# FifthEpoch/longcat-video-tta

Hardware: AMD Instinct MI355X
Metric: denoised latent frames/sec (49x720p, 50-step CFG denoise) (higher is better)
Workload: dtype bf16; 1 GPU; K3: 49x720p (13 latent frames, 46 800 tokens); DiT 48 blocks x 4096 hidden, CFG 4.0, 50-step flow-match Euler, no conditioning frames; depth=48, parallelism=dp1

## Files before the change

longcat-video-tta_amd/csrc/attn_fwd_w64.hip:

```cpp
#include "attn_common.h"
#include <type_traits>

struct AttnFwdW64Params : AttnFwdLead {
  float scale;
  int gx, xcd_remap;
};

template <int I, int N, class F>
__device__ __forceinline__ void w64_static_for(F&& f) {
  if constexpr (I < N) { f(std::integral_constant<int, I>{}); w64_static_for<I + 1, N>(f); }
}
enum : unsigned char { W64_NONE, W64_EXP, W64_ADD, W64_PACK, W64_LRUN, W64_VOFF, W64_MAX, W64_HMAX, W64_BALLOT, W64_M0, W64_DMA };
struct W64Op { unsigned char kind, b, e; };
constexpr int W64_SLOTS = 6;
constexpr W64Op W64_P1[32][W64_SLOTS] = {
  {{W64_EXP, 0, 0}, {W64_EXP, 1, 0}},
  {{W64_EXP, 0, 1}},
  {{W64_PACK, 0, 0}, {W64_ADD, 0, 1}, {W64_EXP, 1, 1}, {W64_EXP, 0, 2}},
  {{W64_ADD, 0, 2}, {W64_PACK, 1, 0}, {W64_ADD, 1, 1}, {W64_EXP, 1, 2}},
  {{W64_ADD, 1, 2}, {W64_EXP, 0, 3}, {W64_EXP, 1, 3}},
  {{W64_PACK, 0, 1}, {W64_ADD, 0, 3}, {W64_PACK, 1, 1}, {W64_ADD, 1, 3}, {W64_EXP, 0, 4}},
  {{W64_ADD, 0, 4}, {W64_EXP, 1, 4}, {W64_EXP, 0, 5}},
  {{W64_PACK, 0, 2}, {W64_ADD, 0, 5}, {W64_ADD, 1, 4}, {W64_EXP, 1, 5}},
  {{W64_PACK, 1, 2}, {W64_ADD, 1, 5}, {W64_EXP, 0, 6}, {W64_EXP, 1, 6}},
  {{W64_ADD, 0, 6}, {W64_ADD, 1, 6}, {W64_EXP, 0, 7}},
  {{W64_VOFF, 0, 0}, {W64_PACK, 0, 3}, {W64_ADD, 0, 7}, {W64_EXP, 1, 7}, {W64_EXP, 0, 8}},
  {{W64_VOFF, 1, 0}, {W64_ADD, 0, 8}, {W64_PACK, 1, 3}, {W64_ADD, 1, 7}, {W64_EXP, 1, 8}},
  {{W64_VOFF, 2, 0}, {W64_ADD, 1, 8}, {W64_EXP, 0, 9}, {W64_EXP, 1, 9}},
  {{W64_VOFF, 3, 0}, {W64_PACK, 0, 4}, {W64_ADD, 0, 9}, {W64_PACK, 1, 4}, {W64_ADD, 1, 9}, {W64_EXP, 0, 10}},
  {{W64_VOFF, 4, 0}, {W64_ADD, 0, 10}, {W64_EXP, 1, 10}, {W64_EXP, 0, 11}},
  {{W64_VOFF, 5, 0}, {W64_PACK, 0, 5}, {W64_ADD, 0, 11}, {W64_ADD, 1, 10}, {W64_EXP, 1, 11}},
  {{W64_VOFF, 6, 0}, {W64_PACK, 1, 5}, {W64_ADD, 1, 11}, {W64_EXP, 0, 12}, {W64_EXP, 1, 12}},
  {{W64_VOFF, 7, 0}, {W64_ADD, 0, 12}, {W64_ADD, 1, 12}, {W64_EXP, 0, 13}},
  {{W64_PACK, 0, 6}, {W64_ADD, 0, 13}, {W64_EXP, 1, 13}, {W64_EXP, 0, 14}},
  {{W64_ADD, 0, 14}, {W64_PACK, 1, 6}, {W64_ADD, 1, 13}, {W64_EXP, 1, 14}},
  {{W64_ADD, 1, 14}, {W64_EXP, 0, 15}, {W64_EXP, 1, 15}},
  {{W64_PACK, 0, 7}, {W64_ADD, 0, 15}, {W64_PACK, 1, 7}, {W64_ADD, 1, 15}, {W64_EXP, 0, 16}},
  {{W64_ADD, 0, 16}, {W64_EXP, 1, 16}, {W64_EXP, 0, 17}},
  {{W64_PACK, 0, 8}, {W64_ADD, 0, 17}, {W64_ADD, 1, 16}, {W64_EXP, 1, 17}},
  {{W64_PACK, 1, 8}, {W64_ADD, 1, 17}, {W64_EXP, 0, 18}, {W64_EXP, 1, 18}},
  {{W64_ADD, 0, 18}, {W64_ADD, 1, 18}, {W64_EXP, 0, 19}},
  {{W64_PACK, 0, 9}, {W64_ADD, 0, 19}, {W64_EXP, 1, 19}, {W64_EXP, 0, 20}},
  {{W64_ADD, 0, 20}, {W64_PACK, 1, 9}, {W64_ADD, 1, 19}, {W64_EXP, 1, 20}},
  {{W64_ADD, 1, 20}, {W64_EXP, 0, 21}, {W64_EXP, 1, 21}},
  {{W64_PACK, 0, 10}, {W64_ADD, 0, 21}, {W64_PACK, 1, 10}, {W64_ADD, 1, 21}, {W64_EXP, 0, 22}},
  {{W64_ADD, 0, 22}, {W64_EXP, 1, 22}, {W64_EXP, 0, 23}},
  {{W64_PACK, 0, 11}, {W64_ADD, 0, 23}, {W64_ADD, 1, 22}, {W64_EXP, 1, 23}},
};
constexpr W64Op W64_P2[32][W64_SLOTS] = {
  {{W64_M0, 0, 0}, {W64_PACK, 1, 11}, {W64_ADD, 1, 23}, {W64_EXP, 0, 24}, {W64_DMA, 0, 0}},
  {{W64_ADD, 0, 24}, {W64_EXP, 1, 24}},
  {{W64_M0, 1, 0}, {W64_ADD, 1, 24}, {W64_EXP, 0, 25}, {W64_DMA, 1, 0}},
  {{W64_PACK, 0, 12}, {W64_ADD, 0, 25}},
  {{W64_M0, 2, 0}, {W64_EXP, 1, 25}, {W64_DMA, 2, 0}},
  {{W64_PACK, 1, 12}, {W64_ADD, 1, 25}, {W64_EXP, 0, 26}},
  {{W64_M0, 3, 0}, {W64_ADD, 0, 26}, {W64_DMA, 3, 0}},
  {{W64_EXP, 1, 26}},
  {{W64_M0, 4, 0}, {W64_ADD, 1, 26}, {W64_MAX, 0, 0}, {W64_EXP, 0, 27}, {W64_DMA, 4, 0}},
  {{W64_PACK, 0, 13}, {W64_ADD, 0, 27}, {W64_MAX, 1, 0}},
  {{W64_M0, 5, 0}, {W64_MAX, 0, 1}, {W64_EXP, 1, 27}, {W64_DMA, 5, 0}},
  {{W64_PACK, 1, 13}, {W64_ADD, 1, 27}, {W64_MAX, 1, 1}, {W64_EXP, 0, 28}},
  {{W64_M0, 6, 0}, {W64_ADD, 0, 28}, {W64_MAX, 0, 2}, {W64_EXP, 1, 28}, {W64_DMA, 6, 0}},
  {{W64_ADD, 1, 28}, {W64_MAX, 1, 2}},
  {{W64_M0, 7, 0}, {W64_MAX, 0, 3}, {W64_EXP, 0, 29}, {W64_DMA, 7, 0}},
  {{W64_PACK, 0, 14}, {W64_ADD, 0, 29}, {W64_MAX, 1, 3}, {W64_EXP, 1, 29}},
  {{W64_PACK, 1, 14}, {W64_ADD, 1, 29}, {W64_MAX, 0, 4}},
  {{W64_MAX, 1, 4}, {W64_EXP, 0, 30}},
  {{W64_ADD, 0, 30}, {W64_MAX, 0, 5}, {W64_EXP, 1, 30}},
  {{W64_ADD, 1, 30}, {W64_MAX, 1, 5}},
  {{W64_MAX, 0, 6}, {W64_EXP, 0, 31}},
  {{W64_PACK, 0, 15}, {W64_ADD, 0, 31}, {W64_MAX, 1, 6}, {W64_EXP, 1, 31}},
  {{W64_PACK, 1, 15}, {W64_ADD, 1, 31}, {W64_LRUN, 0, 0}, {W64_MAX, 0, 7}},
  {{W64_LRUN, 1, 0}, {W64_MAX, 1, 7}},
  {{W64_HMAX, 0, 0}},
  {{W64_HMAX, 1, 0}},
  {{W64_BALLOT, 0, 0}},
  {{W64_BALLOT, 1, 0}},
  {},
  {},
  {},
  {},
};
constexpr int w64_op_cost(W64Op o) {
  return o.kind == W64_EXP ? 8 : o.kind == W64_PACK ? 5 : o.kind == W64_MAX ? 8 : o.kind == W64_HMAX ? 20 :
         o.kind == W64_NONE ? 0 : 4;
}
constexpr int w64_read_cost(int phase, int i) {
  return !(i & 1) || i > 29 ? 0 : ((phase == 1 && i >= 27) || (phase == 2 && i <= 25)) ? 12 : 8;
}
constexpr bool w64_table_ok(const W64Op (&t)[32][W64_SLOTS], int phase, int max_cyc, int max_exp) {
  for (int i = 0; i < 32; ++i) {
    int c = w64_read_cost(phase, i), ex = 0;
    for (int s = 0; s < W64_SLOTS; ++s) { c += w64_op_cost(t[i][s]); ex += t[i][s].kind == W64_EXP; }
    if (c > max_cyc || ex > max_exp) return false;
  }
  return true;
}
constexpr bool w64_table_complete() {
  int exp_at[2][32] = {}, add_at[2][32] = {}, pack_at[2][16] = {}, n = 0;
  for (int b = 0; b < 2; ++b) for (int e = 0; e < 32; ++e) { exp_at[b][e] = -1; add_at[b][e] = -1; }
  for (int b = 0; b < 2; ++b) for (int m = 0; m < 16; ++m) pack_at[b][m] = -1;
  for (int g = 0; g < 64; ++g)
    for (int s = 0; s < W64_SLOTS; ++s) {
      const W64Op o = g < 32 ? W64_P1[g][s] : W64_P2[g - 32][s];
      const int at = 8 * g + s;
      if (o.kind == W64_EXP) { if (exp_at[o.b][o.e] >= 0) return false; exp_at[o.b][o.e] = at; ++n; }
      if (o.kind == W64_ADD) { if (o.e == 0 || exp_at[o.b][o.e] < 0 || (o.e > 1 && add_at[o.b][o.e - 1] < 0)) return false; add_at[o.b][o.e] = at; }
      if (o.kind == W64_PACK) { if (exp_at[o.b][2 * o.e] < 0 || exp_at[o.b][2 * o.e + 1] < 0) return false; pack_at[o.b][o.e] = at; }
      if (o.kind == W64_LRUN && add_at[o.b][31] < 0) return false;
    }
  for (int b = 0; b < 2; ++b)
    for (int m = 0; m < 16; ++m)
      if (pack_at[b][m] < 0 || pack_at[b][m] >= 8 * (32 + 8 * (m / 4) + b - 1) + W64_SLOTS) return false;
  return n == 64;
}
static_assert(w64_table_complete(), "attn_fwd_w64 gap table: an exp, add or pack is missing, doubled or out of order");
static_assert(w64_table_ok(W64_P1, 1, 38, 2) && w64_table_ok(W64_P2, 2, 37, 1), "attn_fwd_w64 gap table over its budget");

template <bool GUARD>
__device__ __forceinline__ void mfma_s(f32x16& c, const bf16x8& a, const bf16x8& b) {
  if constexpr (GUARD) asm volatile("s_nop 3\n\tv_mfma_f32_32x32x16_bf16 %0, %1, %2, %0" : "+v"(c) : "v"(a), "a"(b));
  else asm volatile("v_mfma_f32_32x32x16_bf16 %0, %1, %2, %0" : "+v"(c) : "v"(a), "a"(b));
}
template <bool GUARD>
__device__ __forceinline__ void mfma_s_first(f32x16& d, const f32x16& c, const bf16x8& a, const bf16x8& b) {
  if constexpr (GUARD) asm volatile("s_nop 3\n\tv_mfma_f32_32x32x16_bf16 %0, %2, %3, %1" : "=&v"(d) : "v"(c), "v"(a), "a"(b));
  else asm volatile("v_mfma_f32_32x32x16_bf16 %0, %2, %3, %1" : "=&v"(d) : "v"(c), "v"(a), "a"(b));
}
template <bool GUARD>
__device__ __forceinline__ void mfma_o(f32x16& c, const bf16x8& a, const bf16x8& b) {
  if constexpr (GUARD) asm volatile("s_nop 3\n\tv_mfma_f32_32x32x16_bf16 %0, %1, %2, %0" : "+a"(c) : "v"(a), "v"(b));
  else asm volatile("v_mfma_f32_32x32x16_bf16 %0, %1, %2, %0" : "+a"(c) : "v"(a), "v"(b));
}

#define SCW(S, nb, j) (S[(j) >> 4][nb][(j) & 15])

__global__ __launch_bounds__(256) void attn_fwd_w64_kernel(const AttnFwdW64Params p) {
  constexpr int TILE = 64 * 256;
  extern __shared__ __attribute__((aligned(16))) unsigned char smem[];
  lds_u8* lds = (lds_u8*)smem;
  constexpr int V_REGION = 2 * TILE;

  const int tid = threadIdx.x;
  const int lane = tid & 63;
  const int wave = __builtin_amdgcn_readfirstlane(tid >> 6);
  const int r = lane & 31, h = lane >> 5;
  int qb, head;
  int64_t b;
  ATTN_BLOCK_DECODE(p, qb, head, b);
  const int64_t q0 = (int64_t)qb * 256 + wave * 64;
  const int nt = (int)((p.d.Nk + 63) / 64);
  const bool ragged = (p.d.Nk & 63) != 0;
  const char* kbase_u = lcv_uniform_ptr(p.k + b * p.d.k_sb + (int64_t)head * p.d.k_sh);
  const char* vbase_u = lcv_uniform_ptr(p.v + b * p.d.v_sb + (int64_t)head * p.d.v_sh);

  auto dma_row_of = [&](int ln, int i) { return 16 * wave + 4 * i + (ln >> 4); };
  auto dma_colb_of = [&](int ln, int i) {
    const int row = dma_row_of(ln, i);
    return 16 * ((ln & 15) ^ attn_swz(row));
  };
  unsigned koff[4], voff[4];
#pragma unroll
  for (int i = 0; i < 4; ++i) {
    koff[i] = (unsigned)(dma_row_of(lane, i) * p.d.k_sn * 2 + dma_colb_of(lane, i));
    voff[i] = (unsigned)(dma_row_of(lane, i) * p.d.v_sn * 2 + dma_colb_of(lane, i));
  }
  auto last_off = [&](int i, int64_t sn) {
    const int ln = lane_now();
    int64_t row = (int64_t)(nt - 1) * 64 + dma_row_of(ln, i);
    if (row > p.d.Nk - 1) row = p.d.Nk - 1;
    return (unsigned)(row * sn * 2 + dma_colb_of(ln, i));
  };
  const unsigned lds_wave = (unsigned)(uintptr_t)lds + (unsigned)wave * 4096u;
  auto dma_one = [&](int which, int i, int dst_tile, int tile, bool known_full) __attribute__((always_inline)) {
    const int64_t sn = which ? p.d.v_sn : p.d.k_sn;
    const char* base = which ? vbase_u : kbase_u;
    unsigned off = which ? voff[i] : koff[i];
    if (!known_full && tile == nt - 1) off = last_off(i, sn);
    else base += (int64_t)tile * (128 * sn);
    asm volatile("s_mov_b32 m0, %2\n\ts_nop 0\n\tglobal_load_lds_dwordx4 %0, %1"
                 :: "v"(off), "s"(base), "s"(lds_wave + (unsigned)dst_tile + 1024u * i) : "memory", "m0");
  };
  auto dma_m0 = [&](int i, int dst_tile) __attribute__((always_inline)) {
    asm volatile("s_mov_b32 m0, %0" :: "s"(lds_wave + (unsigned)dst_tile + 1024u * i) : "memory", "m0");
  };
  auto dma_req = [&](int which, int i, int tile, bool known_full) __attribute__((always_inline)) {
    const int64_t sn = which ? p.d.v_sn : p.d.k_sn;
    const char* base = which ? vbase_u : kbase_u;
    unsigned off = which ? voff[i] : koff[i];
    if (!known_full && tile == nt - 1) off = last_off(i, sn);
    else base += (int64_t)tile * (128 * sn);
    asm volatile("global_load_lds_dwordx4 %0, %1" :: "v"(off), "s"(base) : "memory");
  };
  auto dma_tile = [&](int which, int dst_tile, int tile) __attribute__((always_inline)) {
#pragma unroll
    for (int i = 0; i < 4; ++i) dma_one(which, i, dst_tile, tile, false);
  };
  constexpr int KOP = 0, VOP = 1;
  auto dma_wait_and_barrier = [&]() { asm volatile("s_waitcnt vmcnt(0)\n\ts_barrier" ::: "memory"); };

  int k_off[8];
  int v_off[2][4];
  auto set_read_offsets = [&](int ln, int slot) {
    const int rr = ln & 31, hh = ln >> 5;
    const int kfz = ((rr & 3) << 2) | ((rr >> 2) & 3);
#pragma unroll
    for (int ks = 0; ks < 8; ++ks) k_off[ks] = 256 * rr + 16 * ((2 * ks + hh) ^ kfz);
    const int q4 = (ln >> 2) & 3, p4 = ln & 3, g1 = (ln >> 4) & 1;
#pragma unroll
    for (int half = 0; half < 2; ++half)
#pragma unroll
      for (int d = 0; d < 4; ++d)
        v_off[half][d] = (int)(unsigned)(uintptr_t)lds + V_REGION + slot * TILE + 256 * (4 * hh + 8 * half + q4) + 8 * (p4 & 1) + 64 * (d ^ q4) +
                         16 * ((2 * g1 + (p4 >> 1)) ^ (hh + 2 * half));
  };
  set_read_offsets(lane, 2);
  auto read_k = [&](const lds_u8* kb, int f) __attribute__((always_inline)) -> bf16x8 {
    return *reinterpret_cast<const AS3 bf16x8*>(kb + (f & 1) * 32 * 256 + k_off[f >> 1]);
  };
  auto read_v = [&](int g) __attribute__((always_inline)) -> bf16x8 {
    const s16x4 lo = __builtin_amdgcn_ds_read_tr16_b64_v4i16((AS3 s16x4*)(uintptr_t)(unsigned)(v_off[0][g & 3] + 4096 * (g >> 2)));
    const s16x4 hi = __builtin_amdgcn_ds_read_tr16_b64_v4i16((AS3 s16x4*)(uintptr_t)(unsigned)(v_off[1][g & 3] + 4096 * (g >> 2)));
    return __builtin_bit_cast(bf16x8, __builtin_shufflevector(lo, hi, 0, 1, 2, 3, 4, 5, 6, 7));
  };

  bf16x8 qf[2][8];
#pragma unroll
  for (int nb = 0; nb < 2; ++nb) {
    int64_t qrow = q0 + 32 * nb + r;
    if (qrow > p.d.Nq - 1) qrow = p.d.Nq - 1;
    const bf16_t* qp = p.q + b * p.d.q_sb + qrow * p.d.q_sn + (int64_t)head * p.d.q_sh + 8 * h;
#pragma unroll
    for (int ks = 0; ks < 8; ++ks) qf[nb][ks] = *reinterpret_cast<const bf16x8*>(qp + 16 * ks);
  }
#pragma unroll
  for (int nb = 0; nb < 2; ++nb)
#pragma unroll
    for (int ks = 0; ks < 8; ++ks) asm volatile("" : "+a"(qf[nb][ks]));

  f32x16 oacc[2][4];
#pragma unroll
  for (int nb = 0; nb < 2; ++nb)
#pragma unroll
    for (int d = 0; d < 4; ++d) {
#pragma unroll
      for (int e = 0; e < 16; ++e) oacc[nb][d][e] = 0.f;
      asm volatile("" : "+a"(oacc[nb][d]));
    }
  float m_run[2] = {0.f, 0.f}, l_run[2] = {0.f, 0.f};
  f32x16 minit[2];
#pragma unroll
  for (int nb = 0; nb < 2; ++nb)
#pragma unroll
    for (int e = 0; e < 16; ++e) minit[nb][e] = 0.f;
  f32x16 sa[2][2], sb[2][2];

  auto mask_last = [&](f32x16 (&s)[2][2]) __attribute__((always_inline)) {
    const int valid = (int)(p.d.Nk - (int64_t)(nt - 1) * 64);
    const int hh_ = lane_now() >> 5;
#pragma unroll
    for (int nb = 0; nb < 2; ++nb)
#pragma unroll
      for (int e = 0; e < 16; ++e) {
        const int key = (e & 3) + 8 * (e >> 2) + 4 * hh_;
        if (key >= valid) s[0][nb][e] = -INFINITY;
        if (key + 32 >= valid) s[1][nb][e] = -INFINITY;
      }
  };
  auto fence_o = [&]() __attribute__((always_inline)) {
    asm volatile("s_nop 15\n\ts_nop 15\n\ts_nop 15\n\ts_nop 15"
                 : "+a"(oacc[0][0]), "+a"(oacc[0][1]), "+a"(oacc[0][2]), "+a"(oacc[0][3]), "+a"(oacc[1][0]), "+a"(oacc[1][1]),
                   "+a"(oacc[1][2]), "+a"(oacc[1][3]));
  };
  auto fence_s = [&](f32x16 (&s)[2][2]) __attribute__((always_inline)) {
    asm volatile("s_nop 15\n\ts_nop 15\n\ts_nop 15\n\ts_nop 15" : "+v"(s[0][0]), "+v"(s[0][1]), "+v"(s[1][0]), "+v"(s[1][1]));
  };
  auto settle = [&](f32x16 (&s)[2][2], auto nb_c, float mx, bool first, bool need) __attribute__((always_inline)) {
    constexpr int nb = decltype(nb_c)::value;
    if (need || first) {
      fence_o();
      const float d = first ? mx : fmaxf(mx, 0.f);
      const float alpha = __builtin_amdgcn_exp2f(-d);
      m_run[nb] += d;
      l_run[nb] *= alpha;
#pragma unroll
      for (int dd = 0; dd < 4; ++dd)
#pragma unroll
        for (int e = 0; e < 16; ++e) oacc[nb][dd][e] *= alpha;
#pragma unroll
      for (int e = 0; e < 16; ++e) {
        s[0][nb][e] -= d;
        s[1][nb][e] -= d;
        asm volatile("v_mov_b32 %0, %1" : "+v"(minit[nb][e]) : "v"(-m_run[nb]));
      }
      fence_o();
    }
  };

#ifndef W64_PD
#define W64_PD 2
#endif
  constexpr int PD = W64_PD, RING = PD + 1;
  bf16x8 kfr[RING], vfr[RING];
  int v_slot = 2;
  auto next_v_slot = [&]() __attribute__((always_inline)) -> int {
    v_slot = (v_slot == 2) ? 0 : v_slot + 1;
    return (v_slot == 0) ? -2 * TILE : TILE;
  };

  dma_tile(KOP, 0, 0);
  dma_tile(VOP, V_REGION, 0);
  dma_tile(KOP, TILE, 1);
  dma_tile(VOP, V_REGION + TILE, 1);
  dma_wait_and_barrier();
  {
#pragma unroll
    for (int kb_ = 0; kb_ < 2; ++kb_)
#pragma unroll
      for (int nb = 0; nb < 2; ++nb)
#pragma unroll
        for (int e = 0; e < 16; ++e) sa[kb_][nb][e] = 0.f;
#pragma unroll
    for (int f = 0; f < 16; ++f) {
      const bf16x8 a = read_k(lds, f);
      mfma_s<true>(sa[f & 1][0], a, qf[0][f >> 1]);
      mfma_s<true>(sa[f & 1][1], a, qf[1][f >> 1]);
    }
    fence_s(sa);
    auto first_settle = [&](auto nb_c) __attribute__((always_inline)) {
      constexpr int nb = decltype(nb_c)::value;
      float mx = sa[0][nb][0];
#pragma unroll
      for (int e = 1; e < 16; ++e) mx = fmaxf(mx, sa[0][nb][e]);
#pragma unroll
      for (int e = 0; e < 16; ++e) mx = fmaxf(mx, sa[1][nb][e]);
      settle(sa, nb_c, half_max(mx), true, true);
    };
    first_settle(std::integral_constant<int, 0>{});
    first_settle(std::integral_constant<int, 1>{});
  }
  __syncthreads();
  dma_tile(KOP, 0, 2);
#pragma unroll
  for (int i = 0; i < PD; ++i) kfr[i] = read_k(lds + TILE, i);

  auto iteration = [&](const int t, auto par_c, auto steady_c, f32x16 (&c)[2][2], f32x16 (&n)[2][2]) __attribute__((always_inline)) {
    constexpr int PAR = decltype(par_c)::value;
    constexpr bool STEADY = decltype(steady_c)::value;
    const lds_u8* kb = lds + (PAR ^ 1) * TILE;
    const lds_u8* kb_next = lds + PAR * TILE;
    const bool has_k3 = STEADY || t + 3 < nt;
    const bool has_v2 = STEADY || t + 2 < nt;
    const int v_delta = next_v_slot();
    const int v_dst = V_REGION + ((v_slot == 0) ? 2 : v_slot - 1) * TILE;
    float psum[2];
    float ex[2][32];
    unsigned pw[2][16];
    float mxa[2] = {0.f, 0.f}, mxb[2] = {0.f, 0.f}, mxh[2] = {0.f, 0.f};
    bool need[2] = {false, false};
    auto run_op = [&](auto phase_c, auto gap_c, auto slot_c) __attribute__((always_inline)) {
      constexpr W64Op o = decltype(phase_c)::value == 1 ? W64_P1[decltype(gap_c)::value][decltype(slot_c)::value]
                                                        : W64_P2[decltype(gap_c)::value][decltype(slot_c)::value];
      constexpr int b_ = o.b, e = o.e;
      if constexpr (o.kind == W64_EXP) ex[b_][e] = gap_exp2(SCW(c, b_, e));
      if constexpr (o.kind == W64_ADD) psum[b_] = gap_add((e == 1) ? ex[b_][0] : psum[b_], ex[b_][e]);
      if constexpr (o.kind == W64_PACK) pw[b_][e] = gap_pack(ex[b_][2 * e], ex[b_][2 * e + 1]);
      if constexpr (o.kind == W64_LRUN) l_run[b_] = gap_add(l_run[b_], psum[b_]);
      if constexpr (o.kind == W64_VOFF) asm volatile("v_add_u32 %0, %1, %0" : "+v"(v_off[b_ >> 2][b_ & 3]) : "s"(v_delta));
      if constexpr (o.kind == W64_MAX) {
        if constexpr (e == 0) {
          mxa[b_] = gap_max3(n[0][b_][0], n[0][b_][1], n[0][b_][2]);
          mxb[b_] = gap_max3(n[1][b_][0], n[1][b_][1], n[1][b_][2]);
        } else if constexpr (e < 7) {
          mxa[b_] = gap_max3(mxa[b_], n[0][b_][2 * e + 1], n[0][b_][2 * e + 2]);
          mxb[b_] = gap_max3(mxb[b_], n[1][b_][2 * e + 1], n[1][b_][2 * e + 2]);
        } else {
          mxa[b_] = gap_max3(mxa[b_], n[0][b_][15], mxb[b_]);
          mxb[b_] = gap_max3(mxa[b_], n[1][b_][15], n[1][b_][14]);
        }
      }
      if constexpr (o.kind == W64_HMAX) mxh[b_] = half_max(mxb[b_]);
      if constexpr (o.kind == W64_BALLOT) need[b_] = __builtin_amdgcn_ballot_w64(mxh[b_] > ATTN_RESCALE_THR) != 0ull;
      if constexpr (o.kind == W64_M0) {
        if constexpr (b_ < 4) { if (has_k3) dma_m0(b_, (PAR ^ 1) * TILE); }
        else { if (has_v2) dma_m0(b_ & 3, v_dst); }
      }
      if constexpr (o.kind == W64_DMA) {
        if constexpr (b_ < 4) { if (has_k3) dma_req(KOP, b_, t + 3, STEADY); }
        else { if (has_v2) dma_req(VOP, b_ & 3, t + 2, STEADY); }
      }
    };
    SCHED_FENCE();
    w64_static_for<0, 32>([&](auto i_c) __attribute__((always_inline)) {
      constexpr int i = decltype(i_c)::value;
      const int f = i >> 1, nb = i & 1;
      if (nb == 0) {
        if (f + PD < 16) kfr[(f + PD) % RING] = read_k(kb, f + PD);
        if (f >= 16 - PD) vfr[f - (16 - PD)] = read_v(f - (16 - PD));
      }
      if (f < 2) {
        if (STEADY && i >= 1) mfma_s_first<false>(n[f & 1][nb], minit[nb], kfr[f % RING], qf[nb][0]);
        else mfma_s_first<true>(n[f & 1][nb], minit[nb], kfr[f % RING], qf[nb][0]);
      } else {
        if (STEADY) mfma_s<false>(n[f & 1][nb], kfr[f % RING], qf[nb][f >> 1]);
        else mfma_s<true>(n[f & 1][nb], kfr[f % RING], qf[nb][f >> 1]);
      }
      SCHED_FENCE();
      w64_static_for<0, W64_SLOTS>([&](auto s_c) { run_op(std::integral_constant<int, 1>{}, i_c, s_c); });
      SCHED_FENCE();
    });
    if constexpr (!STEADY) {
      fence_s(n);
      if (t + 1 == nt - 1 && ragged) mask_last(n);
    }
    dma_wait_and_barrier();
    SCHED_FENCE();
    w64_static_for<0, 32>([&](auto j_c) __attribute__((always_inline)) {
      constexpr int j = decltype(j_c)::value;
      const int g = j >> 1, nb = j & 1;
      if (nb == 0) {
        if (g + PD < 16) vfr[(g + PD) % RING] = read_v(g + PD);
        if (g >= 16 - PD) kfr[g - (16 - PD)] = read_k(kb_next, g - (16 - PD));
      }
      const int kk = g >> 2;
      const u32x4 pbw = {pw[nb][4 * kk], pw[nb][4 * kk + 1], pw[nb][4 * kk + 2], pw[nb][4 * kk + 3]};
      if (STEADY && j >= 2) mfma_o<false>(oacc[nb][g & 3], vfr[g % RING], __builtin_bit_cast(bf16x8, pbw));
      else mfma_o<true>(oacc[nb][g & 3], vfr[g % RING], __builtin_bit_cast(bf16x8, pbw));
      SCHED_FENCE();
      w64_static_for<0, W64_SLOTS>([&](auto s_c) { run_op(std::integral_constant<int, 2>{}, j_c, s_c); });
      SCHED_FENCE();
    });
    settle(n, std::integral_constant<int, 0>{}, mxh[0], false, need[0]);
    settle(n, std::integral_constant<int, 1>{}, mxh[1], false, need[1]);
  };

  auto final_tile = [&](f32x16 (&c)[2][2]) __attribute__((always_inline)) {
    const int v_delta = next_v_slot();
#pragma unroll
    for (int i = 0; i < 8; ++i) v_off[i >> 2][i & 3] += v_delta;
    unsigned pw[2][16];
#pragma unroll
    for (int nb = 0; nb < 2; ++nb) {
      float psum = 0.f;
      float ex[32];
#pragma unroll
      for (int j = 0; j < 32; ++j) {
        ex[j] = __builtin_amdgcn_exp2f(SCW(c, nb, j));
        psum += ex[j];
      }
      l_run[nb] += psum;
#pragma unroll
      for (int m = 0; m < 16; ++m) pw[nb][m] = gap_pack(ex[2 * m], ex[2 * m + 1]);
    }
#pragma unroll
    for (int g = 0; g < 16; ++g) {
      const bf16x8 vf_ = read_v(g);
      const int kk = g >> 2;
#pragma unroll
      for (int nb = 0; nb < 2; ++nb) {
        const u32x4 pbw = {pw[nb][4 * kk], pw[nb][4 * kk + 1], pw[nb][4 * kk + 2], pw[nb][4 * kk + 3]};
        mfma_o<true>(oacc[nb][g & 3], vf_, __builtin_bit_cast(bf16x8, pbw));
      }
    }
    fence_o();
  };

  {
    using P0 = std::integral_constant<int, 0>;
    using P1 = std::integral_constant<int, 1>;
    int t = 0;
    for (; t + 5 < nt; t += 2) {
      iteration(t, P0{}, std::true_type{}, sa, sb);
      iteration(t + 1, P1{}, std::true_type{}, sb, sa);
    }
    fence_o(); fence_s(sa); fence_s(sb);
    for (; t + 1 <= nt - 2; t += 2) {
      iteration(t, P0{}, std::false_type{}, sa, sb);
      iteration(t + 1, P1{}, std::false_type{}, sb, sa);
    }
    if (t == nt - 2) iteration(t, P0{}, std::false_type{}, sa, sb);
    fence_o(); fence_s(sa); fence_s(sb);
    set_read_offsets(lane_now(), v_slot);
    if ((nt - 1) & 1) final_tile(sb);
    else final_tile(sa);
  }

  const int lane_l = lane_now();
  const int r_l = lane_l & 31, h_l = lane_l >> 5;
#pragma unroll
  for (int nb = 0; nb < 2; ++nb) {
    const float l_tot = half_sum(l_run[nb]);
    const float inv = 1.0f / l_tot;
    const int64_t qrow = q0 + 32 * nb + r_l;
    if (qrow < p.d.Nq) {
      bf16_t* op = p.o + b * p.d.o_sb + qrow * p.d.o_sn + (int64_t)head * p.d.o_sh;
#pragma unroll
      for (int d = 0; d < 4; ++d)
#pragma unroll
        for (int i = 0; i < 4; ++i) {
          u16x4 pk;
#pragma unroll
          for (int e = 0; e < 4; ++e) pk[e] = f2bf(oacc[nb][d][4 * i + e] * inv);
          *reinterpret_cast<u16x4*>(op + 32 * d + 8 * i + 4 * h_l) = pk;
        }
      if (p.lse && h_l == 0) p.lse[(b * p.d.H + head) * p.d.Nq + qrow] = m_run[nb] * p.scale + __logf(l_tot);
    }
  }
}

int attn_fwd_w64_launch(const AttnArgs& a, bool xcd_ok, hipStream_t s) {
  const AttnGrid g = attn_grid(a.B, a.H, (a.Nq + 255) / 256, xcd_ok);
  const AttnFwdW64Params p = {attn_fwd_lead(a), a.scale, g.gx, g.xcd_remap};
  const size_t lds = 5 * 64 * 256;
  ATTN_RAISE_LDS_ONCE("attn_fwd_w64", attn_raise_lds((const void*)attn_fwd_w64_kernel, lds));
  hipLaunchKernelGGL(attn_fwd_w64_kernel, g.grid, dim3(256), lds, s, p);
  LCV_LAUNCH_CHECK("attn_fwd_w64");
  return LCV_OK;
}
```

Measured before the change: 0.06296 latent frames/s.

## Move LDS fragment reads into odd MFMA gaps and split final max op

Shifts the K/V LDS fragment reads from before the even-slot MFMA to after the odd-slot MFMA, so each read issues right behind a matrix op and its latency is hidden by the following gap. The last row-max step is split into two half-cost ops spread over two gaps. The compile-time table checker gains a rule that an op may not sit in the gap right after the value it consumes unless a read or wait separates them. The aim is fewer stalls on LDS reads and dependent VALU chains inside the softmax/MFMA interleave, at the cost of a more complex schedule and a prefetch that moves one slot later.

```diff
diff --git a/longcat-video-tta_amd/csrc/attn_fwd_w64.hip b/longcat-video-tta_amd/csrc/attn_fwd_w64.hip
--- a/longcat-video-tta_amd/csrc/attn_fwd_w64.hip
+++ b/longcat-video-tta_amd/csrc/attn_fwd_w64.hip
@@ -71,8 +71,8 @@
   {{W64_MAX, 0, 6}, {W64_EXP, 0, 31}},
   {{W64_PACK, 0, 15}, {W64_ADD, 0, 31}, {W64_MAX, 1, 6}, {W64_EXP, 1, 31}},
   {{W64_PACK, 1, 15}, {W64_ADD, 1, 31}, {W64_LRUN, 0, 0}, {W64_MAX, 0, 7}},
-  {{W64_LRUN, 1, 0}, {W64_MAX, 1, 7}},
-  {{W64_HMAX, 0, 0}},
+  {{W64_LRUN, 1, 0}, {W64_MAX, 0, 8}, {W64_MAX, 1, 7}},
+  {{W64_MAX, 1, 8}, {W64_HMAX, 0, 0}},
   {{W64_HMAX, 1, 0}},
   {{W64_BALLOT, 0, 0}},
   {{W64_BALLOT, 1, 0}},
@@ -82,11 +82,14 @@
   {},
 };
 constexpr int w64_op_cost(W64Op o) {
-  return o.kind == W64_EXP ? 8 : o.kind == W64_PACK ? 5 : o.kind == W64_MAX ? 8 : o.kind == W64_HMAX ? 20 :
+  return o.kind == W64_EXP ? 8 : o.kind == W64_PACK ? 5 : o.kind == W64_MAX ? (o.e < 7 ? 8 : 4) : o.kind == W64_HMAX ? 20 :
          o.kind == W64_NONE ? 0 : 4;
 }
+constexpr bool w64_read_first(int phase, int i) { return (i & 1) && (phase == 1 || i <= 29); }
+constexpr bool w64_wait_last(int phase, int i) { return (i & 1) && (phase == 1 || i <= 29); }
 constexpr int w64_read_cost(int phase, int i) {
-  return !(i & 1) || i > 29 ? 0 : ((phase == 1 && i >= 27) || (phase == 2 && i <= 25)) ? 12 : 8;
+  const bool v = phase == 1 ? i >= 27 : i <= 25;
+  return (w64_read_first(phase, i) ? (v ? 8 : 4) : 0) + (w64_wait_last(phase, i) && i <= 29 ? 4 : 0);
 }
 constexpr bool w64_table_ok(const W64Op (&t)[32][W64_SLOTS], int phase, int max_cyc, int max_exp) {
   for (int i = 0; i < 32; ++i) {
@@ -96,8 +99,17 @@
   }
   return true;
 }
+constexpr bool w64_apart(int from, int to) {
+  const int gf = from / 8, gt = to / 8;
+  for (int g = gf; g <= gt; ++g) {
+    const int ph = g < 32 ? 1 : 2, i = g & 31;
+    if ((g > gf && w64_read_first(ph, i)) || (g < gt && w64_wait_last(ph, i))) return true;
+  }
+  return false;
+}
 constexpr bool w64_table_complete() {
-  int exp_at[2][32] = {}, add_at[2][32] = {}, pack_at[2][16] = {}, n = 0;
+  int exp_at[2][32] = {}, add_at[2][32] = {}, pack_at[2][16] = {}, max_at[2][9] = {}, n = 0;
+  for (int b = 0; b < 2; ++b) for (int m = 0; m < 9; ++m) max_at[b][m] = -1;
   for (int b = 0; b < 2; ++b) for (int e = 0; e < 32; ++e) { exp_at[b][e] = -1; add_at[b][e] = -1; }
   for (int b = 0; b < 2; ++b) for (int m = 0; m < 16; ++m) pack_at[b][m] = -1;
   for (int g = 0; g < 64; ++g)
@@ -108,13 +120,20 @@
       if (o.kind == W64_ADD) { if (o.e == 0 || exp_at[o.b][o.e] < 0 || (o.e > 1 && add_at[o.b][o.e - 1] < 0)) return false; add_at[o.b][o.e] = at; }
       if (o.kind == W64_PACK) { if (exp_at[o.b][2 * o.e] < 0 || exp_at[o.b][2 * o.e + 1] < 0) return false; pack_at[o.b][o.e] = at; }
       if (o.kind == W64_LRUN && add_at[o.b][31] < 0) return false;
+      if (o.kind == W64_MAX) { if (o.e > 0 && max_at[o.b][o.e - 1] < 0) return false; max_at[o.b][o.e] = at; }
+      if (o.kind == W64_HMAX && max_at[o.b][8] < 0) return false;
+      if (o.kind == W64_ADD && !(w64_apart(exp_at[o.b][o.e], at) && w64_apart(o.e == 1 ? exp_at[o.b][0] : add_at[o.b][o.e - 1], at))) return false;
+      if (o.kind == W64_PACK && !(w64_apart(exp_at[o.b][2 * o.e], at) && w64_apart(exp_at[o.b][2 * o.e + 1], at))) return false;
+      if (o.kind == W64_LRUN && !w64_apart(add_at[o.b][31], at)) return false;
+      if (o.kind == W64_MAX && o.e > 0 && !w64_apart(max_at[o.b][o.e - 1], at)) return false;
+      if (o.kind == W64_HMAX && !w64_apart(max_at[o.b][8], at)) return false;
     }
   for (int b = 0; b < 2; ++b)
     for (int m = 0; m < 16; ++m)
       if (pack_at[b][m] < 0 || pack_at[b][m] >= 8 * (32 + 8 * (m / 4) + b - 1) + W64_SLOTS) return false;
   return n == 64;
 }
-static_assert(w64_table_complete(), "attn_fwd_w64 gap table: an exp, add or pack is missing, doubled or out of order");
+static_assert(w64_table_complete(), "attn_fwd_w64 gap table: an exp, add or pack is missing, doubled, out of order or right behind what it reads");
 static_assert(w64_table_ok(W64_P1, 1, 38, 2) && w64_table_ok(W64_P2, 2, 37, 1), "attn_fwd_w64 gap table over its budget");
 
 template <bool GUARD>
@@ -374,8 +393,9 @@
         } else if constexpr (e < 7) {
           mxa[b_] = gap_max3(mxa[b_], n[0][b_][2 * e + 1], n[0][b_][2 * e + 2]);
           mxb[b_] = gap_max3(mxb[b_], n[1][b_][2 * e + 1], n[1][b_][2 * e + 2]);
+        } else if constexpr (e == 7) {
+          mxa[b_] = gap_max3(mxa[b_], n[0][b_][15], mxb[b_]);
         } else {
-          mxa[b_] = gap_max3(mxa[b_], n[0][b_][15], mxb[b_]);
           mxb[b_] = gap_max3(mxa[b_], n[1][b_][15], n[1][b_][14]);
         }
       }
@@ -394,10 +414,7 @@
     w64_static_for<0, 32>([&](auto i_c) __attribute__((always_inline)) {
       constexpr int i = decltype(i_c)::value;
       const int f = i >> 1, nb = i & 1;
-      if (nb == 0) {
-        if (f + PD < 16) kfr[(f + PD) % RING] = read_k(kb, f + PD);
-        if (f >= 16 - PD) vfr[f - (16 - PD)] = read_v(f - (16 - PD));
-      }
+      if (i == 0) kfr[PD % RING] = read_k(kb, PD);
       if (f < 2) {
         if (STEADY && i >= 1) mfma_s_first<false>(n[f & 1][nb], minit[nb], kfr[f % RING], qf[nb][0]);
         else mfma_s_first<true>(n[f & 1][nb], minit[nb], kfr[f % RING], qf[nb][0]);
@@ -406,6 +423,13 @@
         else mfma_s<true>(n[f & 1][nb], kfr[f % RING], qf[nb][f >> 1]);
       }
       SCHED_FENCE();
+      if (nb == 1) {
+        const int fn = f + 1;
+        if (fn + PD < 16) kfr[(fn + PD) % RING] = read_k(kb, fn + PD);
+        else if (fn < 16) vfr[fn - (16 - PD)] = read_v(fn - (16 - PD));
+        else vfr[PD % RING] = read_v(PD);
+        SCHED_FENCE();
+      }
       w64_static_for<0, W64_SLOTS>([&](auto s_c) { run_op(std::integral_constant<int, 1>{}, i_c, s_c); });
       SCHED_FENCE();
     });
@@ -418,15 +442,17 @@
     w64_static_for<0, 32>([&](auto j_c) __attribute__((always_inline)) {
       constexpr int j = decltype(j_c)::value;
       const int g = j >> 1, nb = j & 1;
-      if (nb == 0) {
-        if (g + PD < 16) vfr[(g + PD) % RING] = read_v(g + PD);
-        if (g >= 16 - PD) kfr[g - (16 - PD)] = read_k(kb_next, g - (16 - PD));
-      }
       const int kk = g >> 2;
       const u32x4 pbw = {pw[nb][4 * kk], pw[nb][4 * kk + 1], pw[nb][4 * kk + 2], pw[nb][4 * kk + 3]};
       if (STEADY && j >= 2) mfma_o<false>(oacc[nb][g & 3], vfr[g % RING], __builtin_bit_cast(bf16x8, pbw));
       else mfma_o<true>(oacc[nb][g & 3], vfr[g % RING], __builtin_bit_cast(bf16x8, pbw));
       SCHED_FENCE();
+      if (nb == 1 && g + 1 < 16) {
+        const int gn = g + 1;
+        if (gn + PD < 16) vfr[(gn + PD) % RING] = read_v(gn + PD);
+        else kfr[gn - (16 - PD)] = read_k(kb_next, gn - (16 - PD));
+        SCHED_FENCE();
+      }
       w64_static_for<0, W64_SLOTS>([&](auto s_c) { run_op(std::integral_constant<int, 2>{}, j_c, s_c); });
       SCHED_FENCE();
     });
```

New measurement: 0.06393 latent frames/s (median of 6 runs). 1.02x the previous value.
